# GuanRunwei/ASY-VRNet

Hardware: AMD Instinct MI355X
Metric: images/sec fwd+bwd, 512x512 img+4ch radar, bs=8/GPU (higher is better)
Workload: dtype f32; 1 GPU; EfficientVRNet(phi=l) forward+backward, 512x512 image + 4x512x512 radar, bs=8/GPU, fp32, det+seg heads (BASELINE.json configs[1]); random weights; global_batch=8, image_size=512, parallelism=dp1, launch=hipgraph

## Files before the change

asy-vrnet_amd/csrc/spatial.hip:

```cpp
#include "common.h"

#include <cstdlib>

namespace {

__global__ __launch_bounds__(256) void dwconv3x3_kernel(const float* x, long ldx, const float* w, float* y, long ldy,
                                                        int B, int H, int W, int C, int flip, int accumulate) {
  const int total = B * H * W * C;
  for (int e = blockIdx.x * 256 + threadIdx.x; e < total; e += gridDim.x * 256) {
    const int c = e % C;
    const int pix = e / C;
    const int xx = pix % W;
    const int q = pix / W;
    const int yy = q % H;
    const int b = q / H;
    float s = 0.f;
#pragma unroll
    for (int ky = 0; ky < 3; ++ky) {
      const int sy = yy + ky - 1;
      if (sy < 0 || sy >= H) continue;
      const float* row = x + ((long)(b * H + sy) * W) * ldx + c;
#pragma unroll
      for (int kx = 0; kx < 3; ++kx) {
        const int sx = xx + kx - 1;
// ... 223 lines not shown
    for (int j = 0; j < 4; ++j)
#pragma unroll
      for (int t = 0; t < 9; ++t) d[j * 9 + t] = acc[t][j];
  }
}
__global__ __launch_bounds__(256) void dwconv3x3_wgrad_reduce_kernel(const float* partial, int nchunks, int C, float* dw,
                                                                     int accumulate) {
  __shared__ double red[16][16];
  const int o = threadIdx.x & 15, sl = threadIdx.x >> 4;
  const int e = blockIdx.x * 16 + o;
  const bool live = e < C * 9;
  double s = 0;
  if (live)
    for (int k = sl; k < nchunks; k += 16) s += partial[(long)k * C * 9 + e];
  red[sl][o] = s;
  __syncthreads();
  if (sl == 0 && live) {
#pragma unroll
    for (int k = 1; k < 16; ++k) s += red[k][o];
    dw[e] = (accumulate ? dw[e] : 0.f) + (float)s;
  }
}

__global__ __launch_bounds__(256) void patch_gather_kernel(const float* x, long ldx, const float* pos, float* out, int B,
                                                           int H, int W, int C, int CP, int k) {
  const int CT = C + CP, KT = k * k * CT, OH = H / k, OW = W / k;
  const long total = (long)B * OH * OW * KT;
  for (long e = (long)blockIdx.x * 256 + threadIdx.x; e < total; e += (long)gridDim.x * 256) {
    const int ch = e % KT;
    const long op = e / KT;
    const int t = ch / CT, c = ch - t * CT;
    const int ky = t / k, kx = t - ky * k;
    const int ox = op % OW;
    const long q = op / OW;
    const int oy = q % OH;
    const long b = q / OH;
    const int yy = oy * k + ky, xx = ox * k + kx;
    out[e] = c < C ? x[((b * H + yy) * W + xx) * ldx + c] : pos[((long)yy * W + xx) * CP + (c - C)];
  }
}
__global__ __launch_bounds__(256) void patch_scatter_kernel(const float* dp, float* dx, long lddx, int B, int H, int W, int C,
                                                            int CP, int k, int accumulate) {
  const int CT = C + CP, KT = k * k * CT, OH = H / k, OW = W / k;
  const long total = (long)B * H * W * C;
  for (long e = (long)blockIdx.x * 256 + threadIdx.x; e < total; e += (long)gridDim.x * 256) {
    const int c = e % C;
    const long pix = e / C;
    const int xx = pix % W;
    const long q = pix / W;
    const int yy = q % H;
    const long b = q / H;
    const int t = (yy % k) * k + (xx % k);
    const float v = dp[((b * OH + yy / k) * OW + xx / k) * KT + t * CT + c];
    float* d = dx + pix * lddx + c;
    *d = accumulate ? *d + v : v;
  }
}
__global__ void ohwi_kernel(const float* src, float* dst, int Cout, int Cin, int T, int dir, int accumulate) {
  const long total = (long)Cout * Cin * T;
  const long e = (long)blockIdx.x * blockDim.x + threadIdx.x;
  if (e >= total) return;
  const int t = e % T;
  const long q = e / T;
  const int c = q % Cin;
  const long n = q / Cin;
  const long oihw = e, ohwi = (n * T + t) * Cin + c;
  if (dir == 0) dst[ohwi] = src[oihw];
  else dst[oihw] = (accumulate ? dst[oihw] : 0.f) + src[ohwi];
}

__device__ __forceinline__ void src_index(float scale, int o, int in_size, int* i0, int* i1, float* l1) {
  const float r = scale * (float)o;
  int a = (int)r;
  if (a > in_size - 1) a = in_size - 1;
  *i0 = a;
  *i1 = a + ((a < in_size - 1) ? 1 : 0);
  *l1 = r - (float)a;
}

__device__ __forceinline__ float up_tap(float v, const float* bnA, const float* bnD, const float* bnS, int c) {
  return bnA ? fmaxf(__builtin_fmaf(bnA[c], v - bnS[c], bnD[c]), 0.f) : v;
}

__global__ __launch_bounds__(256) void upsample_kernel(const float* x, long ldx, float* y, long ldy, int B, int H,
                                                       int W, int C, int OH, int OW, int out_nchw, const float* bnA,
                                                       const float* bnD, const float* bnS) {
  const float ry = OH > 1 ? (float)(H - 1) / (float)(OH - 1) : 0.f;
  const float rx = OW > 1 ? (float)(W - 1) / (float)(OW - 1) : 0.f;
  const long total = (long)B * OH * OW * C;
  for (long e = (long)blockIdx.x * 256 + threadIdx.x; e < total; e += (long)gridDim.x * 256) {
    int c, ox, oy;
    long b;
    if (out_nchw) {
      ox = e % OW; long q = e / OW; oy = q % OH; q /= OH; c = q % C; b = q / C;
    } else {
      c = e % C; long q = e / C; ox = q % OW; q /= OW; oy = q % OH; b = q / OH;
    }
    int y0, y1, x0, x1;
    float ly, lx;
    src_index(ry, oy, H, &y0, &y1, &ly);
    src_index(rx, ox, W, &x0, &x1, &lx);
    const float* base = x + (b * H * W) * ldx + c;
    const float v00 = up_tap(base[((long)y0 * W + x0) * ldx], bnA, bnD, bnS, c), v01 = up_tap(base[((long)y0 * W + x1) * ldx], bnA, bnD, bnS, c);
    const float v10 = up_tap(base[((long)y1 * W + x0) * ldx], bnA, bnD, bnS, c), v11 = up_tap(base[((long)y1 * W + x1) * ldx], bnA, bnD, bnS, c);
    const float v = (1.f - ly) * ((1.f - lx) * v00 + lx * v01) + ly * ((1.f - lx) * v10 + lx * v11);
    if (out_nchw) y[e] = v;
    else y[((b * OH + oy) * OW + ox) * ldy + c] = v;
  }
}

__global__ __launch_bounds__(256) void upsample_vec_kernel(const float* x, long ldx, float* y, long ldy, int B, int H, int W,
                                                           int C, int OH, int OW, const float* bnA, const float* bnD,
                                                           const float* bnS) {
  const float ry = OH > 1 ? (float)(H - 1) / (float)(OH - 1) : 0.f;
  const float rx = OW > 1 ? (float)(W - 1) / (float)(OW - 1) : 0.f;
  const int CQ = C >> 2;
  const long total = (long)B * OH * OW * CQ;
  for (long e = (long)blockIdx.x * 256 + threadIdx.x; e < total; e += (long)gridDim.x * 256) {
    const int cq = e % CQ;
    long q = e / CQ;
    const int ox = q % OW; q /= OW;
    const int oy = q % OH;
    const long b = q / OH;
    int y0, y1, x0, x1;
    float ly, lx;
    src_index(ry, oy, H, &y0, &y1, &ly);
    src_index(rx, ox, W, &x0, &x1, &lx);
    const float* base = x + (b * H * W) * ldx + 4 * cq;
    f32x4 v00 = *reinterpret_cast<const f32x4*>(base + ((long)y0 * W + x0) * ldx);
    f32x4 v01 = *reinterpret_cast<const f32x4*>(base + ((long)y0 * W + x1) * ldx);
    f32x4 v10 = *reinterpret_cast<const f32x4*>(base + ((long)y1 * W + x0) * ldx);
    f32x4 v11 = *reinterpret_cast<const f32x4*>(base + ((long)y1 * W + x1) * ldx);
    if (bnA) {
#pragma unroll
      for (int j = 0; j < 4; ++j) {
        const int c = 4 * cq + j;
        v00[j] = up_tap(v00[j], bnA, bnD, bnS, c);
        v01[j] = up_tap(v01[j], bnA, bnD, bnS, c);
        v10[j] = up_tap(v10[j], bnA, bnD, bnS, c);
        v11[j] = up_tap(v11[j], bnA, bnD, bnS, c);
      }
    }
    f32x4 v;
#pragma unroll
    for (int j = 0; j < 4; ++j) v[j] = (1.f - ly) * ((1.f - lx) * v00[j] + lx * v01[j]) + ly * ((1.f - lx) * v10[j] + lx * v11[j]);
    *reinterpret_cast<f32x4*>(y + ((b * OH + oy) * OW + ox) * ldy + 4 * cq) = v;
  }
}

__global__ __launch_bounds__(256) void upsample_bwd_vec_kernel(const float* dy, long lddy, float* dx, long lddx, int B, int H,
                                                               int W, int C, int OH, int OW, int accumulate) {
  const float ry = OH > 1 ? (float)(H - 1) / (float)(OH - 1) : 0.f;
  const float rx = OW > 1 ? (float)(W - 1) / (float)(OW - 1) : 0.f;
  const int CQ = C >> 2;
  const long total = (long)B * H * W * CQ;
  for (long e = (long)blockIdx.x * 256 + threadIdx.x; e < total; e += (long)gridDim.x * 256) {
    const int cq = e % CQ;
    long q = e / CQ;
    const int ix = q % W; q /= W;
    const int iy = q % H;
    const long b = q / H;
    int oy_lo = 0, oy_hi = OH - 1, ox_lo = 0, ox_hi = OW - 1;
    if (ry > 0.f) {
      oy_lo = max(0, (int)floorf((float)(iy - 1) / ry) - 1);
      oy_hi = min(OH - 1, (int)ceilf((float)(iy + 1) / ry) + 1);
    }
    if (rx > 0.f) {
      ox_lo = max(0, (int)floorf((float)(ix - 1) / rx) - 1);
      ox_hi = min(OW - 1, (int)ceilf((float)(ix + 1) / rx) + 1);
    }
    f32x4 s = {0.f, 0.f, 0.f, 0.f};
    for (int oy = oy_lo; oy <= oy_hi; ++oy) {
      int y0, y1;
      float ly;
      src_index(ry, oy, H, &y0, &y1, &ly);
      const float wy = (y0 == iy ? 1.f - ly : 0.f) + (y1 == iy ? ly : 0.f);
      if (wy == 0.f) continue;
      for (int ox = ox_lo; ox <= ox_hi; ++ox) {
        int x0, x1;
        float lx;
        src_index(rx, ox, W, &x0, &x1, &lx);
        const float wx = (x0 == ix ? 1.f - lx : 0.f) + (x1 == ix ? lx : 0.f);
        if (wx == 0.f) continue;
        const f32x4 g = *reinterpret_cast<const f32x4*>(dy + ((b * OH + oy) * (long)OW + ox) * lddy + 4 * cq);
        const float w = wy * wx;
#pragma unroll
        for (int j = 0; j < 4; ++j) s[j] += w * g[j];
      }
    }
    f32x4* d = reinterpret_cast<f32x4*>(dx + ((b * H + iy) * (long)W + ix) * lddx + 4 * cq);
    if (accumulate) s += *d;
    *d = s;
  }
}

__global__ __launch_bounds__(256) void upsample_nchw4_kernel(const float* x, long ldx, float* y, int B, int H, int W, int C,
                                                             int OH, int OW, const float* bnA, const float* bnD,
                                                             const float* bnS) {
  const float ry = OH > 1 ? (float)(H - 1) / (float)(OH - 1) : 0.f;
  const float rx = OW > 1 ? (float)(W - 1) / (float)(OW - 1) : 0.f;
  const int OQ = OW >> 2;
  const long total = (long)B * C * OH * OQ;
  for (long e = (long)blockIdx.x * 256 + threadIdx.x; e < total; e += (long)gridDim.x * 256) {
    const int oq = e % OQ;
    long q = e / OQ;
    const int oy = q % OH; q /= OH;
    const int c = q % C;
    const long b = q / C;
    int y0, y1;
    float ly;
    src_index(ry, oy, H, &y0, &y1, &ly);
    const float* r0 = x + ((b * H + y0) * (long)W) * ldx + c;
    const float* r1 = x + ((b * H + y1) * (long)W) * ldx + c;
    f32x4 v;
#pragma unroll
    for (int j = 0; j < 4; ++j) {
      int x0, x1;
      float lx;
      src_index(rx, 4 * oq + j, W, &x0, &x1, &lx);
      const float v00 = up_tap(r0[(long)x0 * ldx], bnA, bnD, bnS, c), v01 = up_tap(r0[(long)x1 * ldx], bnA, bnD, bnS, c);
      const float v10 = up_tap(r1[(long)x0 * ldx], bnA, bnD, bnS, c), v11 = up_tap(r1[(long)x1 * ldx], bnA, bnD, bnS, c);
      v[j] = (1.f - ly) * ((1.f - lx) * v00 + lx * v01) + ly * ((1.f - lx) * v10 + lx * v11);
    }
    *reinterpret_cast<f32x4*>(y + ((b * C + c) * OH + oy) * (long)OW + 4 * oq) = v;
  }
}

__global__ __launch_bounds__(256) void upsample_bwd_kernel(const float* dy, long lddy, int dy_nchw, float* dx, long lddx,
                                                           int B, int H, int W, int C, int OH, int OW, int accumulate) {
  const float ry = OH > 1 ? (float)(H - 1) / (float)(OH - 1) : 0.f;
  const float rx = OW > 1 ? (float)(W - 1) / (float)(OW - 1) : 0.f;
  const long total = (long)B * H * W * C;
  for (long e = (long)blockIdx.x * 256 + threadIdx.x; e < total; e += (long)gridDim.x * 256) {
    int c, ix, iy;
    long b;
    if (dy_nchw) {
      ix = e % W;
      long q = e / W;
      iy = q % H; q /= H;
      c = q % C;
      b = q / C;
    } else {
      c = e % C;
      long q = e / C;
      ix = q % W; q /= W;
      iy = q % H;
      b = q / H;
    }
    int oy_lo = 0, oy_hi = OH - 1, ox_lo = 0, ox_hi = OW - 1;
    if (ry > 0.f) {
      oy_lo = max(0, (int)floorf((float)(iy - 1) / ry) - 1);
      oy_hi = min(OH - 1, (int)ceilf((float)(iy + 1) / ry) + 1);
    }
    if (rx > 0.f) {
      ox_lo = max(0, (int)floorf((float)(ix - 1) / rx) - 1);
      ox_hi = min(OW - 1, (int)ceilf((float)(ix + 1) / rx) + 1);
    }
    float s = 0.f;
    constexpr int MAXR = 16;
    const int nx = ox_hi - ox_lo + 1;
    float wxs[MAXR];
    if (nx <= MAXR) {
#pragma unroll
      for (int t = 0; t < MAXR; ++t) {
        int x0, x1;
        float lx;
        src_index(rx, min(ox_lo + t, OW - 1), W, &x0, &x1, &lx);
        wxs[t] = t < nx ? (x0 == ix ? 1.f - lx : 0.f) + (x1 == ix ? lx : 0.f) : 0.f;
      }
    }
    for (int oy = oy_lo; oy <= oy_hi; ++oy) {
      int y0, y1;
      float ly;
      src_index(ry, oy, H, &y0, &y1, &ly);
      const float wy = (y0 == iy ? 1.f - ly : 0.f) + (y1 == iy ? ly : 0.f);
      if (wy == 0.f) continue;
      if (nx <= MAXR) {
        const float* grow = dy_nchw ? dy + ((b * C + c) * OH + oy) * (long)OW + ox_lo : dy + ((b * OH + oy) * (long)OW + ox_lo) * lddy + c;
        const long gstep = dy_nchw ? 1 : lddy;
#pragma unroll
        for (int t = 0; t < MAXR; ++t) {
          const float wx = wxs[t];
          if (wx == 0.f) continue;
          s += wy * wx * grow[t * gstep];
        }
        continue;
      }
      for (int ox = ox_lo; ox <= ox_hi; ++ox) {
        int x0, x1;
        float lx;
        src_index(rx, ox, W, &x0, &x1, &lx);
        const float wx = (x0 == ix ? 1.f - lx : 0.f) + (x1 == ix ? lx : 0.f);
        if (wx == 0.f) continue;
        const float g = dy_nchw ? dy[((b * C + c) * OH + oy) * (long)OW + ox]
                                : dy[((b * OH + oy) * (long)OW + ox) * lddy + c];
        s += wy * wx * g;
      }
    }
    float* d = dx + ((b * H + iy) * (long)W + ix) * lddx + c;
    *d = accumulate ? *d + s : s;
  }
}

__global__ __launch_bounds__(256) void minmax_partial_kernel(const float* p, long n, float* partial) {
  __shared__ float smn[4], smx[4];
  float mn = INFINITY, mx = -INFINITY;
  for (long e = (long)blockIdx.x * 256 + threadIdx.x; e < n; e += (long)gridDim.x * 256) {
    const float v = p[e];
    mn = fminf(mn, v);
    mx = fmaxf(mx, v);
  }
#pragma unroll
  for (int o = 32; o > 0; o >>= 1) {
    mn = fminf(mn, __shfl_xor(mn, o, 64));
    mx = fmaxf(mx, __shfl_xor(mx, o, 64));
  }
  if ((threadIdx.x & 63) == 0) {
    smn[threadIdx.x >> 6] = mn;
    smx[threadIdx.x >> 6] = mx;
  }
  __syncthreads();
  if (threadIdx.x == 0) {
    partial[2 * blockIdx.x] = fminf(fminf(smn[0], smn[1]), fminf(smn[2], smn[3]));
    partial[2 * blockIdx.x + 1] = fmaxf(fmaxf(smx[0], smx[1]), fmaxf(smx[2], smx[3]));
// ... 286 lines not shown
                                                           const float* P, const float* Q, const float* Mn, const float* E,
                                                           const float* F, float* dx, long lddx, long HW, int C,
                                                           int accumulate) {
  const long b = blockIdx.y;
  const long total = HW * C;
  for (long e = (long)blockIdx.x * 256 + threadIdx.x; e < total; e += (long)gridDim.x * 256) {
    const long r = e / C;
    const int q = e - r * C;
    const float xv = x[(b * HW + r) * ldx + q];
    const float pq = P[b * C + q], mq = Mn[b * C + q];
    const float sg = vr_sigmoid(pq * (xv - mq) + Q[b * C + q]);
    const float g = dy[(b * HW + r) * lddy + sa_dst(q, C)];
    const float v = g * (sg + xv * sg * (1.f - sg) * pq) + E[b * C + q] * (xv - mq) + F[b * C + q];
    float* d = dx + (b * HW + r) * lddx + q;
    *d = accumulate ? *d + v : v;
  }
}

inline long grid_for(long n, long per_block = 1024, long cap = 8192) {
  long g = vr_cdiv(n, per_block);
  return g < 1 ? 1 : (g > cap ? cap : g);
}

void sa_plan(long HW, int C, int* TPR, int* ncb, int* nchunks, long* rows) {
  int t = 1;
  while (t < C && t < 256) t <<= 1;
  *TPR = t;
  *ncb = (int)vr_cdiv(C, t);
  long nc = vr_cdiv(HW * C, 8192);
  if (nc < 1) nc = 1;
  if (nc > 1024) nc = 1024;
  if (nc > HW) nc = HW;
  *rows = vr_cdiv(HW, nc);
  *nchunks = (int)vr_cdiv(HW, *rows);
}

}

extern "C" int vrnet_dwconv3x3_f32(const float* x, long ldx, const float* w, float* y, long ldy, int B, int H, int W,
                                   int C, int flip, int accumulate, void* stream) {
  if (vr_ablated("dwconv")) return VR_OK;
  VR_CHECK_ARG(x && w && y && B > 0 && H > 0 && W > 0 && C > 0, "dwconv3x3: bad arguments");
  VR_CHECK_ARG((long)B * H * W * C < (1L << 31), "dwconv3x3: tensor too large");
  const bool vec = C % 4 == 0 && C <= 1024 && 256 % (C / 4) == 0 && ldx % 4 == 0 && ldy % 4 == 0 && vr_aligned16(x) &&
                   vr_aligned16(y) && vr_aligned16(w);
  static const int slide = vr_tune("VRNET_DW_SLIDE", 1);
// ... 49 lines not shown
    vr_set_error("dwconv3x3_wgrad: workspace too small");
    return VR_ERR_WORKSPACE;
  }
  const int TPR = C <= 32 ? 32 : 64;
  float* partial = reinterpret_cast<float*>(workspace);
  hipStream_t st = vr_stream(stream);
  if (dw_wgrad_slide_ok(W, C, ldx, lddy, x, dy) && vr_tune("VRNET_DW_WGRAD_SLIDE", 1)) {
    const int quads = C / 4 < 64 ? C / 4 : 64, groups = 256 / quads;
    hipLaunchKernelGGL(dwconv3x3_wgrad_slide_kernel, dim3(nchunks, (C / 4) / quads), dim3(256), (size_t)(groups - 1) * quads * 9 * 16, st,
                       x, ldx, dy, lddy, B, H, W, C, (int)ppc, partial);
  } else {
    hipLaunchKernelGGL(dwconv3x3_wgrad_kernel, dim3(nchunks, vr_cdiv(C, TPR)), dim3(256), 0, st, x, ldx, dy, lddy, B, H, W,
                       C, ppc, partial);
  }
  VR_LAUNCH_CHECK("dwconv3x3_wgrad");
  hipLaunchKernelGGL(dwconv3x3_wgrad_reduce_kernel, dim3(vr_cdiv(C * 9, 16)), dim3(256), 0, st, partial, nchunks, C, dw,
                     accumulate);
  VR_LAUNCH_CHECK("dwconv3x3_wgrad_reduce");
  return VR_OK;
}

static int upsample_launch(const float* x, long ldx, float* y, long ldy, int B, int H, int W, int C, int scale, int out_nchw,
                           const float* bnA, const float* bnD, const float* bnS, void* stream) {
  if (!out_nchw && C % 4 == 0 && ldx % 4 == 0 && ldy % 4 == 0 && vr_aligned16(x) && vr_aligned16(y))
    hipLaunchKernelGGL(upsample_vec_kernel, dim3(grid_for((long)B * H * W * scale * scale * (C / 4))), dim3(256), 0,
                       vr_stream(stream), x, ldx, y, ldy, B, H, W, C, H * scale, W * scale, bnA, bnD, bnS);
  else if (out_nchw && (W * scale) % 4 == 0 && vr_aligned16(y))
    hipLaunchKernelGGL(upsample_nchw4_kernel, dim3(grid_for((long)B * H * W * scale * scale * C / 4)), dim3(256), 0,
                       vr_stream(stream), x, ldx, y, B, H, W, C, H * scale, W * scale, bnA, bnD, bnS);
  else
    hipLaunchKernelGGL(upsample_kernel, dim3(grid_for((long)B * H * W * scale * scale * C)), dim3(256), 0,
                       vr_stream(stream), x, ldx, y, ldy, B, H, W, C, H * scale, W * scale, out_nchw, bnA, bnD, bnS);
  VR_LAUNCH_CHECK("upsample");
  return VR_OK;
}

extern "C" int vrnet_upsample_bilinear_f32(const float* x, long ldx, float* y, long ldy, int B, int H, int W, int C,
                                           int scale, int out_nchw, void* stream) {
  if (vr_ablated("misc")) return VR_OK;
  VR_CHECK_ARG(x && y && scale >= 1 && B > 0 && H > 0 && W > 0 && C > 0, "upsample: bad arguments");
  return upsample_launch(x, ldx, y, ldy, B, H, W, C, scale, out_nchw, nullptr, nullptr, nullptr, stream);
}

extern "C" int vrnet_bn_relu_upsample_bilinear_f32(const float* z, long ldz, const float* A, const float* D, const float* S,
                                                   float* y, long ldy, int B, int H, int W, int C, int scale, int out_nchw,
                                                   void* stream) {
  if (vr_ablated("misc")) return VR_OK;
  VR_CHECK_ARG(z && A && D && S && y && scale >= 1 && B > 0 && H > 0 && W > 0 && C > 0, "bn_relu_upsample: bad arguments");
  return upsample_launch(z, ldz, y, ldy, B, H, W, C, scale, out_nchw, A, D, S, stream);
}

extern "C" int vrnet_upsample_bilinear_bwd_f32(const float* dy, long lddy, int dy_nchw, float* dx, long lddx, int B,
                                               int H, int W, int C, int scale, int accumulate, void* stream) {
  if (vr_ablated("misc")) return VR_OK;
  VR_CHECK_ARG(dy && dx && scale >= 1, "upsample_bwd: bad arguments");
  if (!dy_nchw && C % 4 == 0 && lddy % 4 == 0 && lddx % 4 == 0 && vr_aligned16(dy) && vr_aligned16(dx))
    hipLaunchKernelGGL(upsample_bwd_vec_kernel, dim3(grid_for((long)B * H * W * (C / 4), 256)), dim3(256), 0, vr_stream(stream),
                       dy, lddy, dx, lddx, B, H, W, C, H * scale, W * scale, accumulate);
  else
    hipLaunchKernelGGL(upsample_bwd_kernel, dim3(grid_for((long)B * H * W * C, 256)), dim3(256), 0, vr_stream(stream), dy,
                       lddy, dy_nchw, dx, lddx, B, H, W, C, H * scale, W * scale, accumulate);
  VR_LAUNCH_CHECK("upsample_bwd");
  return VR_OK;
}

extern "C" long vrnet_reduce_workspace(void) { return 8192L * 4 * 8 + 256; }

extern "C" int vrnet_minmax_f32(const float* p, long n, float* mm, void* workspace, long workspace_bytes, void* stream) {
  VR_CHECK_ARG(p && mm && workspace && n > 0, "minmax: bad arguments");
  VR_CHECK_ARG(workspace_bytes >= vrnet_reduce_workspace(), "minmax: workspace too small");
  const int nb = (int)grid_for(n, 2048, 2048);
  float* partial = reinterpret_cast<float*>(workspace);
  hipLaunchKernelGGL(minmax_partial_kernel, dim3(nb), dim3(256), 0, vr_stream(stream), p, n, partial);
  VR_LAUNCH_CHECK("minmax_partial");
  hipLaunchKernelGGL(minmax_final_kernel, dim3(1), dim3(256), 0, vr_stream(stream), partial, nb, mm);
  VR_LAUNCH_CHECK("minmax_final");
  return VR_OK;
}

extern "C" int vrnet_enhance_mul_f32(const float* p, const float* x, const float* mm, float* out, long n, void* stream) {
  VR_CHECK_ARG(p && x && mm && out && n > 0, "enhance_mul: bad arguments");
  hipLaunchKernelGGL(enhance_mul_kernel, dim3(grid_for(n)), dim3(256), 0, vr_stream(stream), p, x, mm, out, n);
  VR_LAUNCH_CHECK("enhance_mul");
  return VR_OK;
// ... 77 lines not shown
  hipLaunchKernelGGL(sa_bwd_reduce_kernel, dim3(nchunks, B, ncb), dim3(256), 256 * 2 * sizeof(double), st, dy, lddy, x,
                     ldx, P, Q, Mn, HW, C, TPR, rows, nchunks, partial);
  VR_LAUNCH_CHECK("sa_bwd_reduce");
  hipLaunchKernelGGL(sa_reduce_chunks_kernel, dim3(vr_cdiv((long)B * C * 2, 16)), dim3(256), 0, st, partial, T, B,
                     nchunks, C);
  VR_LAUNCH_CHECK("sa_reduce_chunks");
  SaParams sp{cw, cb, sw, sb, gnw, gnb};
  const int nb1 = (int)vr_cdiv((long)B * C, 256);
  float* E = EF;
  float* F = EF + (long)B * C;
  hipLaunchKernelGGL(sa_coef_bwd_kernel, dim3(nb1 + C / (2 * G)), dim3(256), 0, st, T, mom, sp, B, HW, C, G, nb1, E, F, dcw, dcb,
                     dsw, dsb, dgnw, dgnb, accumulate_params);
  VR_LAUNCH_CHECK("sa_coef_bwd");
  hipLaunchKernelGGL(sa_bwd_apply_kernel, dim3(grid_for(HW * C), B), dim3(256), 0, st, dy, lddy, x, ldx, P, Q, Mn, E, F, dx,
                     lddx, HW, C, accumulate_dx);
  VR_LAUNCH_CHECK("sa_bwd_apply");
  return VR_OK;
}

extern "C" int vrnet_patch_gather_f32(const float* x, long ldx, const float* pos, float* out, int B, int H, int W, int C,
                                      int CP, int k, void* stream) {
  VR_CHECK_ARG(x && out && (CP == 0 || pos) && B > 0 && C > 0 && CP >= 0 && k > 0 && H % k == 0 && W % k == 0 && ldx >= C,
               "patch_gather: bad arguments");
  hipLaunchKernelGGL(patch_gather_kernel, dim3(grid_for((long)B * H * W * (C + CP))), dim3(256), 0, vr_stream(stream), x,
                     ldx, pos, out, B, H, W, C, CP, k);
  VR_LAUNCH_CHECK("patch_gather");
  return VR_OK;
}

extern "C" int vrnet_patch_scatter_f32(const float* dp, float* dx, long lddx, int B, int H, int W, int C, int CP, int k,
                                       int accumulate, void* stream) {
  VR_CHECK_ARG(dp && dx && B > 0 && C > 0 && CP >= 0 && k > 0 && H % k == 0 && W % k == 0 && lddx >= C,
               "patch_scatter: bad arguments");
  hipLaunchKernelGGL(patch_scatter_kernel, dim3(grid_for((long)B * H * W * C)), dim3(256), 0, vr_stream(stream), dp, dx,
                     lddx, B, H, W, C, CP, k, accumulate);
  VR_LAUNCH_CHECK("patch_scatter");
  return VR_OK;
}

extern "C" int vrnet_weight_ohwi_f32(const float* src, float* dst, int Cout, int Cin, int kh, int kw, int dir,
                                     int accumulate, void* stream) {
  VR_CHECK_ARG(src && dst && Cout > 0 && Cin > 0 && kh > 0 && kw > 0 && (dir == 0 || dir == 1), "weight_ohwi: bad arguments");
  const long total = (long)Cout * Cin * kh * kw;
  hipLaunchKernelGGL(ohwi_kernel, dim3(vr_cdiv(total, 256)), dim3(256), 0, vr_stream(stream), src, dst, Cout, Cin, kh * kw,
                     dir, accumulate);
  VR_LAUNCH_CHECK("weight_ohwi");
  return VR_OK;
}
```

asy-vrnet_amd/csrc/tinyconv.hip:

```cpp
#include "common.h"

namespace tiny {

constexpr int CMAX = 8;

struct Args {
  const float* a; long lda; const float* w; const float* bias; float* y; long ldy;
  int B, H, W, Cin, Cout, k, pad, dil, accumulate;
};

template <int MODE>
__global__ __launch_bounds__(256) void conv_kernel(const Args p) {
  __shared__ float ws[9 * CMAX * CMAX];
  const int T = p.k * p.k;
  for (int i = threadIdx.x; i < T * p.Cout * p.Cin; i += 256) ws[i] = p.w[i];
  __syncthreads();
  const int CK = MODE == 0 ? p.Cin : p.Cout, CN = MODE == 0 ? p.Cout : p.Cin;
  const long total = (long)p.B * p.H * p.W;
  for (long pix = (long)blockIdx.x * 256 + threadIdx.x; pix < total; pix += (long)gridDim.x * 256) {
    const int x = pix % p.W;
    const long q = pix / p.W;
    const int y = q % p.H;
    const long b = q / p.H;
    float acc[CMAX];
// ... 224 lines not shown
  for (int n = 0; n < NO; ++n) {
#pragma unroll
    for (int c = 0; c < CP; ++c)
#pragma unroll
      for (int t = 0; t < T; ++t) {
        const float sum = row16(acc[n][c][t]);
        if (lead) red[rowid][n * NA + c * T + t] = sum;
      }
    const float b = row16(bs[n]);
    if (lead) red[rowid][n * NA + CP * T] = b;
  }
  __syncthreads();
  const int per = Cin * T + 1;
  for (int i = threadIdx.x; i < NO * per; i += 256) {
    const int n = i / per, j = i - n * per;
    const int src = n * NA + (j == Cin * T ? CP * T : j);
    float sum = 0.f;
#pragma unroll
    for (int r = 0; r < 16; ++r) sum += red[r][src];
    partial[((long)blockIdx.x * NO + n) * per + j] = sum;
  }
}

__global__ __launch_bounds__(256) void wgrad_reduce_kernel(const float* partial, int nblk, int Cin, int Cout, int T,
                                                           const float* row_scale, float* dw, float* db, int accumulate) {
  __shared__ double red[16][16];
  const int per = Cin * T + 1;
  const int o = threadIdx.x & 15, sl = threadIdx.x >> 4;
  const int e = blockIdx.x * 16 + o;
  const bool live = e < Cout * per;
  const int n = live ? e / per : 0, i = e - n * per;
  double s = 0;
  if (live)
    for (int b = sl; b < nblk; b += 16) s += partial[((long)b * Cout + n) * per + i];
  red[sl][o] = s;
  __syncthreads();
  if (sl != 0 || !live) return;
#pragma unroll
  for (int k = 1; k < 16; ++k) s += red[k][o];
  float v = (float)s;
  if (row_scale) v *= row_scale[n];
  if (i == Cin * T) {
    if (db) db[n] = accumulate ? db[n] + v : v;
  } else {
    float* d = dw + (long)n * Cin * T + i;
    *d = accumulate ? *d + v : v;
  }
}

__global__ __launch_bounds__(256) void patch_dgrad_kernel(const float* dy, long lddy, const float* w, float* dx, long lddx,
                                                          int B, int H, int W, int Cin, int Cout, int k, int accumulate) {
  extern __shared__ float wsm[];
  const int T = k * k;
  for (int i = threadIdx.x; i < T * Cout * Cin; i += 256) wsm[i] = w[i];
  __syncthreads();
  const int OW = W / k, OH = H / k;
  const long total = (long)B * H * W;
  for (long pix = (long)blockIdx.x * 256 + threadIdx.x; pix < total; pix += (long)gridDim.x * 256) {
    const int x = pix % W;
    const long q = pix / W;
    const int y = q % H;
    const long b = q / H;
    const int t = (y % k) * k + (x % k);
// ... 29 lines not shown
    VR_LAUNCH_CHECK("tiny_conv");                                                                                  \
    return VR_OK;                                                                                                  \
  } while (0)
  if (al && mode == 0) {
    if (Cin == 3 && Cout == 3 && k == 1) VR_TINY_FIXED(0, 3, 3, 1);
    if (Cin == 4 && Cout == 4 && k == 1) VR_TINY_FIXED(0, 4, 4, 1);
    if (Cin == 7 && Cout == 4 && k == 1) VR_TINY_FIXED(0, 7, 4, 1);
    if (Cin == 4 && Cout == 3 && k == 3) VR_TINY_FIXED(0, 4, 3, 3);
  } else if (al) {
    if (Cin == 7 && Cout == 4 && k == 1) VR_TINY_FIXED(1, 4, 7, 1);
    if (Cin == 4 && Cout == 3 && k == 3) VR_TINY_FIXED(1, 3, 4, 3);
    if (Cin == 4 && Cout == 4 && k == 1) VR_TINY_FIXED(1, 4, 4, 1);
    if (Cin == 3 && Cout == 3 && k == 1) VR_TINY_FIXED(1, 3, 3, 1);
  }
#undef VR_TINY_FIXED
  if (mode == 0) hipLaunchKernelGGL((tiny::conv_kernel<0>), dim3(blocks), dim3(256), 0, st, p);
  else hipLaunchKernelGGL((tiny::conv_kernel<1>), dim3(blocks), dim3(256), 0, st, p);
  VR_LAUNCH_CHECK("tiny_conv");
  return VR_OK;
}

static void tiny_wgrad_plan(long npix, int* nblk, long* ppb) {
  long nb = vr_cdiv(npix, 1024);
  if (nb > 2048) nb = 2048;
  if (nb < 1) nb = 1;
  *ppb = vr_cdiv(npix, nb);
  *nblk = (int)vr_cdiv(npix, *ppb);
}

long vr_tiny_wgrad_workspace(long npix, int Cin, int Cout, int T) {
  int nblk;
  long ppb;
  tiny_wgrad_plan(npix, &nblk, &ppb);
  return (long)nblk * Cout * (Cin * T + 1) * 4 + 256;
}

int vr_tiny_wgrad(const float* x, long ldx, const float* dy, long lddy, float* dw, float* db, const float* row_scale,
                  int B, int H, int W, int Cin, int Cout, int k, int pad, int dil, int accumulate, void* workspace,
                  hipStream_t st) {
  int nblk;
  long ppb;
  tiny_wgrad_plan((long)B * H * W, &nblk, &ppb);
  float* partial = reinterpret_cast<float*>(workspace);
  const int vec4 = Cin == 4 && ldx % 4 == 0 && vr_aligned16(x);
  dim3 grid(nblk, Cout), block(256);
#define VR_TINY_WGRAD_ALL(CP_, KS_, NO_)                                                                                 \
  do {                                                                                                                   \
    hipLaunchKernelGGL((tiny::wgrad_all_kernel<CP_, KS_, NO_>), dim3(nblk), block, 0, st, x, ldx, dy, lddy, B, H, W, Cin, pad, \
                       dil, vec4, ppb, partial);                                                                         \
    goto reduce;                                                                                                         \
  } while (0)
  if (k == 3 && Cin == 4 && Cout == 3) VR_TINY_WGRAD_ALL(4, 3, 3);
  if (k == 1 && Cin == 7 && Cout == 4) VR_TINY_WGRAD_ALL(8, 1, 4);
  if (k == 1 && Cin == 4 && Cout == 4) VR_TINY_WGRAD_ALL(4, 1, 4);
  if (k == 1 && Cin == 3 && Cout == 3) VR_TINY_WGRAD_ALL(4, 1, 3);
#undef VR_TINY_WGRAD_ALL
#define VR_TINY_WGRAD(CP_, KS_)                                                                                          \
  hipLaunchKernelGGL((tiny::wgrad_kernel<CP_, KS_>), grid, block, 0, st, x, ldx, dy, lddy, B, H, W, Cin, Cout, pad, dil, vec4, \
                     ppb, partial)
  if (k == 1) {
    if (Cin <= 4) VR_TINY_WGRAD(4, 1);
    else VR_TINY_WGRAD(8, 1);
  } else {
    if (Cin <= 4) VR_TINY_WGRAD(4, 3);
    else VR_TINY_WGRAD(8, 3);
  }
#undef VR_TINY_WGRAD
reduce:
  VR_LAUNCH_CHECK("tiny_wgrad");
  const int per = Cin * k * k + 1;
  hipLaunchKernelGGL(tiny::wgrad_reduce_kernel, dim3(vr_cdiv(Cout * per, 16)), dim3(256), 0, st, partial, nblk, Cin, Cout,
                     k * k, row_scale, dw, db, accumulate);
  VR_LAUNCH_CHECK("tiny_wgrad_reduce");
  return VR_OK;
}

int vr_patch_dgrad(const float* dy, long lddy, const float* w, float* dx, long lddx, int B, int H, int W, int Cin,
                   int Cout, int k, int accumulate, hipStream_t st) {
  long blocks = vr_cdiv((long)B * H * W, 256);
  if (blocks > 16384) blocks = 16384;
  const size_t lds = (size_t)k * k * Cout * Cin * sizeof(float);
  hipLaunchKernelGGL(tiny::patch_dgrad_kernel, dim3(blocks), dim3(256), lds, st, dy, lddy, w, dx, lddx, B, H, W, Cin, Cout,
                     k, accumulate);
  VR_LAUNCH_CHECK("patch_dgrad");
  return VR_OK;
}
```

Baseline: 326.3 images/sec.

## Row-structured indexing for upsample/patch kernels and block-per-output wgrad reduce

Replaces flat grid-stride loops with 64-bit div/mod decomposition in the patch gather/scatter and bilinear upsample forward/backward kernels by a row/item iteration helper that uses 32-bit unsigned index math and fewer divisions. The upsample backward kernels also tighten the contributing output range by trimming zero-weight taps, cache horizontal weights in a smaller fixed array, and use FMA. The tiny-conv weight-gradient reduce now assigns one block per output element, with a wave-level sum instead of a 16x16 shared-memory layout. The point is to cut integer-division overhead and improve coalescing. In exchange it adds argument checks limiting sizes to 2^31 elements and changes floating-point rounding through the explicit FMA usage.

```diff
diff --git a/asy-vrnet_amd/csrc/spatial.hip b/asy-vrnet_amd/csrc/spatial.hip
--- a/asy-vrnet_amd/csrc/spatial.hip
+++ b/asy-vrnet_amd/csrc/spatial.hip
@@ -269,39 +269,47 @@
   }
 }
 
+template <int IPT = 4, class F>
+__device__ __forceinline__ void for_row_items(unsigned rows, unsigned n, F f) {
+  constexpr unsigned CH = 256 * IPT;
+  const unsigned rp = n >= 256 ? 1 : 256 / n;
+  const unsigned nc = (n + CH - 1) / CH;
+  const unsigned sub = threadIdx.x / n, i0 = threadIdx.x - sub * n;
+  if (sub >= rp) return;
+  const unsigned nblk = ((rows + rp - 1) / rp) * nc;
+  for (unsigned blk = blockIdx.x; blk < nblk; blk += gridDim.x) {
+    const unsigned rg = blk / nc, chunk = blk - rg * nc;
+    const unsigned row = rg * rp + sub;
+    if (row >= rows) continue;
+    const unsigned i1 = min(n, (chunk + 1) * CH);
+    for (unsigned i = chunk * CH + i0; i < i1; i += 256) f(row, i);
+  }
+}
+
 __global__ __launch_bounds__(256) void patch_gather_kernel(const float* x, long ldx, const float* pos, float* out, int B,
                                                            int H, int W, int C, int CP, int k) {
-  const int CT = C + CP, KT = k * k * CT, OH = H / k, OW = W / k;
-  const long total = (long)B * OH * OW * KT;
-  for (long e = (long)blockIdx.x * 256 + threadIdx.x; e < total; e += (long)gridDim.x * 256) {
-    const int ch = e % KT;
-    const long op = e / KT;
-    const int t = ch / CT, c = ch - t * CT;
-    const int ky = t / k, kx = t - ky * k;
-    const int ox = op % OW;
-    const long q = op / OW;
-    const int oy = q % OH;
-    const long b = q / OH;
-    const int yy = oy * k + ky, xx = ox * k + kx;
-    out[e] = c < C ? x[((b * H + yy) * W + xx) * ldx + c] : pos[((long)yy * W + xx) * CP + (c - C)];
-  }
+  const unsigned CT = C + CP, KT = k * k * CT, OH = H / k, OW = W / k;
+  for_row_items(B * OH, OW * KT, [&](unsigned row, unsigned i) {
+    const unsigned b = row / OH, oy = row - b * OH;
+    const unsigned ox = i / KT, ch = i - ox * KT;
+    const unsigned t = ch / CT, c = ch - t * CT;
+    const unsigned ky = t / k, kx = t - ky * k;
+    const unsigned yy = oy * k + ky, xx = ox * k + kx;
+    out[(long)row * (OW * KT) + i] = c < (unsigned)C ? x[(((long)b * H + yy) * W + xx) * ldx + c] : pos[((long)yy * W + xx) * CP + (c - C)];
+  });
 }
 __global__ __launch_bounds__(256) void patch_scatter_kernel(const float* dp, float* dx, long lddx, int B, int H, int W, int C,
                                                             int CP, int k, int accumulate) {
-  const int CT = C + CP, KT = k * k * CT, OH = H / k, OW = W / k;
-  const long total = (long)B * H * W * C;
-  for (long e = (long)blockIdx.x * 256 + threadIdx.x; e < total; e += (long)gridDim.x * 256) {
-    const int c = e % C;
-    const long pix = e / C;
-    const int xx = pix % W;
-    const long q = pix / W;
-    const int yy = q % H;
-    const long b = q / H;
-    const int t = (yy % k) * k + (xx % k);
-    const float v = dp[((b * OH + yy / k) * OW + xx / k) * KT + t * CT + c];
-    float* d = dx + pix * lddx + c;
+  const unsigned CT = C + CP, KT = k * k * CT, OH = H / k, OW = W / k;
+  for_row_items(B * H, W * C, [&](unsigned row, unsigned i) {
+    const unsigned b = row / H, yy = row - b * H;
+    const unsigned xx = i / C, c = i - xx * C;
+    const unsigned oy = yy / k, ox = xx / k;
+    const unsigned t = (yy - oy * k) * k + (xx - ox * k);
+    const float v = dp[(((long)b * OH + oy) * OW + ox) * KT + t * CT + c];
+    float* d = dx + ((long)row * W + xx) * lddx + c;
     *d = accumulate ? *d + v : v;
-  }
+  });
 }
 __global__ void ohwi_kernel(const float* src, float* dst, int Cout, int Cin, int T, int dir, int accumulate) {
   const long total = (long)Cout * Cin * T;
@@ -316,13 +324,21 @@
   else dst[oihw] = (accumulate ? dst[oihw] : 0.f) + src[ohwi];
 }
 
+template <bool FUSED>
 __device__ __forceinline__ void src_index(float scale, int o, int in_size, int* i0, int* i1, float* l1) {
+#pragma clang fp contract(off)
   const float r = scale * (float)o;
   int a = (int)r;
   if (a > in_size - 1) a = in_size - 1;
   *i0 = a;
   *i1 = a + ((a < in_size - 1) ? 1 : 0);
-  *l1 = r - (float)a;
+  *l1 = FUSED ? __builtin_fmaf(scale, (float)o, -(float)a) : r - (float)a;
+}
+__device__ __forceinline__ float up_blend(float ly, float lx, float v00, float v01, float v10, float v11) {
+#pragma clang fp contract(off)
+  const float top = __builtin_fmaf(1.f - lx, v00, lx * v01);
+  const float bot = __builtin_fmaf(1.f - lx, v10, lx * v11);
+  return __builtin_fmaf(1.f - ly, top, ly * bot);
 }
 
 __device__ __forceinline__ float up_tap(float v, const float* bnA, const float* bnD, const float* bnS, int c) {
@@ -334,26 +350,25 @@
                                                        const float* bnD, const float* bnS) {
   const float ry = OH > 1 ? (float)(H - 1) / (float)(OH - 1) : 0.f;
   const float rx = OW > 1 ? (float)(W - 1) / (float)(OW - 1) : 0.f;
-  const long total = (long)B * OH * OW * C;
-  for (long e = (long)blockIdx.x * 256 + threadIdx.x; e < total; e += (long)gridDim.x * 256) {
-    int c, ox, oy;
-    long b;
+  for_row_items(out_nchw ? B * C * OH : B * OH, out_nchw ? OW : OW * C, [&](unsigned row, unsigned i) {
+    unsigned c, ox, oy, b;
     if (out_nchw) {
-      ox = e % OW; long q = e / OW; oy = q % OH; q /= OH; c = q % C; b = q / C;
+      const unsigned q = row / OH;
+      oy = row - q * OH; b = q / C; c = q - b * C; ox = i;
     } else {
-      c = e % C; long q = e / C; ox = q % OW; q /= OW; oy = q % OH; b = q / OH;
+      b = row / OH; oy = row - b * OH; ox = i / C; c = i - ox * C;
     }
     int y0, y1, x0, x1;
     float ly, lx;
-    src_index(ry, oy, H, &y0, &y1, &ly);
-    src_index(rx, ox, W, &x0, &x1, &lx);
-    const float* base = x + (b * H * W) * ldx + c;
+    src_index<false>(ry, oy, H, &y0, &y1, &ly);
+    src_index<false>(rx, ox, W, &x0, &x1, &lx);
+    const float* base = x + ((long)b * H * W) * ldx + c;
     const float v00 = up_tap(base[((long)y0 * W + x0) * ldx], bnA, bnD, bnS, c), v01 = up_tap(base[((long)y0 * W + x1) * ldx], bnA, bnD, bnS, c);
     const float v10 = up_tap(base[((long)y1 * W + x0) * ldx], bnA, bnD, bnS, c), v11 = up_tap(base[((long)y1 * W + x1) * ldx], bnA, bnD, bnS, c);
-    const float v = (1.f - ly) * ((1.f - lx) * v00 + lx * v01) + ly * ((1.f - lx) * v10 + lx * v11);
-    if (out_nchw) y[e] = v;
-    else y[((b * OH + oy) * OW + ox) * ldy + c] = v;
-  }
+    const float v = up_blend(ly, lx, v00, v01, v10, v11);
+    if (out_nchw) y[(long)row * OW + ox] = v;
+    else y[((long)row * OW + ox) * ldy + c] = v;
+  });
 }
 
 __global__ __launch_bounds__(256) void upsample_vec_kernel(const float* x, long ldx, float* y, long ldy, int B, int H, int W,
@@ -361,19 +376,15 @@
                                                            const float* bnS) {
   const float ry = OH > 1 ? (float)(H - 1) / (float)(OH - 1) : 0.f;
   const float rx = OW > 1 ? (float)(W - 1) / (float)(OW - 1) : 0.f;
-  const int CQ = C >> 2;
-  const long total = (long)B * OH * OW * CQ;
-  for (long e = (long)blockIdx.x * 256 + threadIdx.x; e < total; e += (long)gridDim.x * 256) {
-    const int cq = e % CQ;
-    long q = e / CQ;
-    const int ox = q % OW; q /= OW;
-    const int oy = q % OH;
-    const long b = q / OH;
+  const unsigned CQ = C >> 2;
+  for_row_items(B * OH, OW * CQ, [&](unsigned row, unsigned i) {
+    const unsigned b = row / OH, oy = row - b * OH;
+    const unsigned ox = i / CQ, cq = i - ox * CQ;
     int y0, y1, x0, x1;
     float ly, lx;
-    src_index(ry, oy, H, &y0, &y1, &ly);
-    src_index(rx, ox, W, &x0, &x1, &lx);
-    const float* base = x + (b * H * W) * ldx + 4 * cq;
+    src_index<false>(ry, oy, H, &y0, &y1, &ly);
+    src_index<false>(rx, ox, W, &x0, &x1, &lx);
+    const float* base = x + ((long)b * H * W) * ldx + 4 * cq;
     f32x4 v00 = *reinterpret_cast<const f32x4*>(base + ((long)y0 * W + x0) * ldx);
     f32x4 v01 = *reinterpret_cast<const f32x4*>(base + ((long)y0 * W + x1) * ldx);
     f32x4 v10 = *reinterpret_cast<const f32x4*>(base + ((long)y1 * W + x0) * ldx);
@@ -390,55 +401,79 @@
     }
     f32x4 v;
 #pragma unroll
-    for (int j = 0; j < 4; ++j) v[j] = (1.f - ly) * ((1.f - lx) * v00[j] + lx * v01[j]) + ly * ((1.f - lx) * v10[j] + lx * v11[j]);
-    *reinterpret_cast<f32x4*>(y + ((b * OH + oy) * OW + ox) * ldy + 4 * cq) = v;
-  }
-}
+    for (int j = 0; j < 4; ++j) v[j] = up_blend(ly, lx, v00[j], v01[j], v10[j], v11[j]);
+    *reinterpret_cast<f32x4*>(y + ((long)row * OW + ox) * ldy + 4 * cq) = v;
+  });
+}
+
+__device__ __forceinline__ float up_weight(float scale, int o, int in_size, int in) {
+  int i0, i1;
+  float l;
+  src_index<true>(scale, o, in_size, &i0, &i1, &l);
+  return (i0 == in ? 1.f - l : 0.f) + (i1 == in ? l : 0.f);
+}
+__device__ __forceinline__ void up_range(float scale, int in, int in_size, int out_size, int* lo, int* hi) {
+  int a = 0, b = out_size - 1;
+  if (scale > 0.f) {
+    a = max(0, (int)floorf((float)(in - 1) / scale) - 1);
+    b = min(out_size - 1, (int)ceilf((float)(in + 1) / scale) + 1);
+  }
+  while (a < b && up_weight(scale, a, in_size, in) == 0.f) ++a;
+  while (b > a && up_weight(scale, b, in_size, in) == 0.f) --b;
+  *lo = a;
+  *hi = b;
+}
+constexpr int UP_MAXR = 12;
 
 __global__ __launch_bounds__(256) void upsample_bwd_vec_kernel(const float* dy, long lddy, float* dx, long lddx, int B, int H,
                                                                int W, int C, int OH, int OW, int accumulate) {
   const float ry = OH > 1 ? (float)(H - 1) / (float)(OH - 1) : 0.f;
   const float rx = OW > 1 ? (float)(W - 1) / (float)(OW - 1) : 0.f;
-  const int CQ = C >> 2;
-  const long total = (long)B * H * W * CQ;
-  for (long e = (long)blockIdx.x * 256 + threadIdx.x; e < total; e += (long)gridDim.x * 256) {
-    const int cq = e % CQ;
-    long q = e / CQ;
-    const int ix = q % W; q /= W;
-    const int iy = q % H;
-    const long b = q / H;
-    int oy_lo = 0, oy_hi = OH - 1, ox_lo = 0, ox_hi = OW - 1;
-    if (ry > 0.f) {
-      oy_lo = max(0, (int)floorf((float)(iy - 1) / ry) - 1);
-      oy_hi = min(OH - 1, (int)ceilf((float)(iy + 1) / ry) + 1);
-    }
-    if (rx > 0.f) {
-      ox_lo = max(0, (int)floorf((float)(ix - 1) / rx) - 1);
-      ox_hi = min(OW - 1, (int)ceilf((float)(ix + 1) / rx) + 1);
+  const unsigned CQ = C >> 2;
+  for_row_items<1>(B * H, W * CQ, [&](unsigned row, unsigned i) {
+    const unsigned b = row / H;
+    const int iy = row - b * H;
+    const unsigned uix = i / CQ, cq = i - uix * CQ;
+    const int ix = uix;
+    int oy_lo, oy_hi, ox_lo, ox_hi;
+    up_range(ry, iy, H, OH, &oy_lo, &oy_hi);
+    up_range(rx, ix, W, OW, &ox_lo, &ox_hi);
+    const int nx = ox_hi - ox_lo + 1;
+    float wxs[UP_MAXR];
+    if (nx <= UP_MAXR) {
+#pragma unroll
+      for (int t = 0; t < UP_MAXR; ++t) wxs[t] = t < nx ? up_weight(rx, min(ox_lo + t, OW - 1), W, ix) : 0.f;
     }
     f32x4 s = {0.f, 0.f, 0.f, 0.f};
     for (int oy = oy_lo; oy <= oy_hi; ++oy) {
-      int y0, y1;
-      float ly;
-      src_index(ry, oy, H, &y0, &y1, &ly);
-      const float wy = (y0 == iy ? 1.f - ly : 0.f) + (y1 == iy ? ly : 0.f);
+      const float wy = up_weight(ry, oy, H, iy);
       if (wy == 0.f) continue;
+      const float* grow = dy + (((long)b * OH + oy) * (long)OW + ox_lo) * lddy + 4 * cq;
+      if (nx <= UP_MAXR) {
+#pragma unroll
+        for (int t = 0; t < UP_MAXR; ++t) {
+          const float wx = wxs[t];
+          if (wx == 0.f) continue;
+          const f32x4 g = *reinterpret_cast<const f32x4*>(grow + t * lddy);
+          const float w = wy * wx;
+#pragma unroll
+          for (int j = 0; j < 4; ++j) s[j] = __builtin_fmaf(w, g[j], s[j]);
+        }
+        continue;
+      }
       for (int ox = ox_lo; ox <= ox_hi; ++ox) {
-        int x0, x1;
-        float lx;
-        src_index(rx, ox, W, &x0, &x1, &lx);
-        const float wx = (x0 == ix ? 1.f - lx : 0.f) + (x1 == ix ? lx : 0.f);
+        const float wx = up_weight(rx, ox, W, ix);
         if (wx == 0.f) continue;
-        const f32x4 g = *reinterpret_cast<const f32x4*>(dy + ((b * OH + oy) * (long)OW + ox) * lddy + 4 * cq);
+        const f32x4 g = *reinterpret_cast<const f32x4*>(grow + (long)(ox - ox_lo) * lddy);
         const float w = wy * wx;
 #pragma unroll
-        for (int j = 0; j < 4; ++j) s[j] += w * g[j];
-      }
-    }
-    f32x4* d = reinterpret_cast<f32x4*>(dx + ((b * H + iy) * (long)W + ix) * lddx + 4 * cq);
+        for (int j = 0; j < 4; ++j) s[j] = __builtin_fmaf(w, g[j], s[j]);
+      }
+    }
+    f32x4* d = reinterpret_cast<f32x4*>(dx + ((long)row * W + ix) * lddx + 4 * cq);
     if (accumulate) s += *d;
     *d = s;
-  }
+  });
 }
 
 __global__ __launch_bounds__(256) void upsample_nchw4_kernel(const float* x, long ldx, float* y, int B, int H, int W, int C,
@@ -446,107 +481,76 @@
                                                              const float* bnS) {
   const float ry = OH > 1 ? (float)(H - 1) / (float)(OH - 1) : 0.f;
   const float rx = OW > 1 ? (float)(W - 1) / (float)(OW - 1) : 0.f;
-  const int OQ = OW >> 2;
-  const long total = (long)B * C * OH * OQ;
-  for (long e = (long)blockIdx.x * 256 + threadIdx.x; e < total; e += (long)gridDim.x * 256) {
-    const int oq = e % OQ;
-    long q = e / OQ;
-    const int oy = q % OH; q /= OH;
-    const int c = q % C;
-    const long b = q / C;
+  for_row_items(B * C * OH, OW >> 2, [&](unsigned row, unsigned oq) {
+    const unsigned q = row / OH, oy = row - q * OH;
+    const unsigned b = q / C, c = q - b * C;
     int y0, y1;
     float ly;
-    src_index(ry, oy, H, &y0, &y1, &ly);
-    const float* r0 = x + ((b * H + y0) * (long)W) * ldx + c;
-    const float* r1 = x + ((b * H + y1) * (long)W) * ldx + c;
+    src_index<false>(ry, oy, H, &y0, &y1, &ly);
+    const float* r0 = x + (((long)b * H + y0) * (long)W) * ldx + c;
+    const float* r1 = x + (((long)b * H + y1) * (long)W) * ldx + c;
     f32x4 v;
 #pragma unroll
     for (int j = 0; j < 4; ++j) {
       int x0, x1;
       float lx;
-      src_index(rx, 4 * oq + j, W, &x0, &x1, &lx);
+      src_index<false>(rx, 4 * oq + j, W, &x0, &x1, &lx);
       const float v00 = up_tap(r0[(long)x0 * ldx], bnA, bnD, bnS, c), v01 = up_tap(r0[(long)x1 * ldx], bnA, bnD, bnS, c);
       const float v10 = up_tap(r1[(long)x0 * ldx], bnA, bnD, bnS, c), v11 = up_tap(r1[(long)x1 * ldx], bnA, bnD, bnS, c);
-      v[j] = (1.f - ly) * ((1.f - lx) * v00 + lx * v01) + ly * ((1.f - lx) * v10 + lx * v11);
-    }
-    *reinterpret_cast<f32x4*>(y + ((b * C + c) * OH + oy) * (long)OW + 4 * oq) = v;
-  }
+      v[j] = up_blend(ly, lx, v00, v01, v10, v11);
+    }
+    *reinterpret_cast<f32x4*>(y + (long)row * OW + 4 * oq) = v;
+  });
 }
 
 __global__ __launch_bounds__(256) void upsample_bwd_kernel(const float* dy, long lddy, int dy_nchw, float* dx, long lddx,
                                                            int B, int H, int W, int C, int OH, int OW, int accumulate) {
   const float ry = OH > 1 ? (float)(H - 1) / (float)(OH - 1) : 0.f;
   const float rx = OW > 1 ? (float)(W - 1) / (float)(OW - 1) : 0.f;
-  const long total = (long)B * H * W * C;
-  for (long e = (long)blockIdx.x * 256 + threadIdx.x; e < total; e += (long)gridDim.x * 256) {
-    int c, ix, iy;
-    long b;
+  for_row_items<1>(dy_nchw ? B * C * H : B * H, dy_nchw ? W : W * C, [&](unsigned row, unsigned i) {
+    unsigned c, b;
+    int ix, iy;
     if (dy_nchw) {
-      ix = e % W;
-      long q = e / W;
-      iy = q % H; q /= H;
-      c = q % C;
-      b = q / C;
+      const unsigned q = row / H;
+      iy = row - q * H; b = q / C; c = q - b * C; ix = i;
     } else {
-      c = e % C;
-      long q = e / C;
-      ix = q % W; q /= W;
-      iy = q % H;
-      b = q / H;
-    }
-    int oy_lo = 0, oy_hi = OH - 1, ox_lo = 0, ox_hi = OW - 1;
-    if (ry > 0.f) {
-      oy_lo = max(0, (int)floorf((float)(iy - 1) / ry) - 1);
-      oy_hi = min(OH - 1, (int)ceilf((float)(iy + 1) / ry) + 1);
-    }
-    if (rx > 0.f) {
-      ox_lo = max(0, (int)floorf((float)(ix - 1) / rx) - 1);
-      ox_hi = min(OW - 1, (int)ceilf((float)(ix + 1) / rx) + 1);
-    }
+      b = row / H; iy = row - b * H;
+      const unsigned uix = i / C;
+      ix = uix; c = i - uix * C;
+    }
+    int oy_lo, oy_hi, ox_lo, ox_hi;
+    up_range(ry, iy, H, OH, &oy_lo, &oy_hi);
+    up_range(rx, ix, W, OW, &ox_lo, &ox_hi);
     float s = 0.f;
-    constexpr int MAXR = 16;
     const int nx = ox_hi - ox_lo + 1;
-    float wxs[MAXR];
-    if (nx <= MAXR) {
-#pragma unroll
-      for (int t = 0; t < MAXR; ++t) {
-        int x0, x1;
-        float lx;
-        src_index(rx, min(ox_lo + t, OW - 1), W, &x0, &x1, &lx);
-        wxs[t] = t < nx ? (x0 == ix ? 1.f - lx : 0.f) + (x1 == ix ? lx : 0.f) : 0.f;
-      }
+    float wxs[UP_MAXR];
+    if (nx <= UP_MAXR) {
+#pragma unroll
+      for (int t = 0; t < UP_MAXR; ++t) wxs[t] = t < nx ? up_weight(rx, min(ox_lo + t, OW - 1), W, ix) : 0.f;
     }
     for (int oy = oy_lo; oy <= oy_hi; ++oy) {
-      int y0, y1;
-      float ly;
-      src_index(ry, oy, H, &y0, &y1, &ly);
-      const float wy = (y0 == iy ? 1.f - ly : 0.f) + (y1 == iy ? ly : 0.f);
+      const float wy = up_weight(ry, oy, H, iy);
       if (wy == 0.f) continue;
-      if (nx <= MAXR) {
-        const float* grow = dy_nchw ? dy + ((b * C + c) * OH + oy) * (long)OW + ox_lo : dy + ((b * OH + oy) * (long)OW + ox_lo) * lddy + c;
-        const long gstep = dy_nchw ? 1 : lddy;
-#pragma unroll
-        for (int t = 0; t < MAXR; ++t) {
+      const float* grow = dy_nchw ? dy + (((long)b * C + c) * OH + oy) * (long)OW + ox_lo : dy + (((long)b * OH + oy) * (long)OW + ox_lo) * lddy + c;
+      const long gstep = dy_nchw ? 1 : lddy;
+      if (nx <= UP_MAXR) {
+#pragma unroll
+        for (int t = 0; t < UP_MAXR; ++t) {
           const float wx = wxs[t];
           if (wx == 0.f) continue;
-          s += wy * wx * grow[t * gstep];
+          s = __builtin_fmaf(wy * wx, grow[t * gstep], s);
         }
         continue;
       }
       for (int ox = ox_lo; ox <= ox_hi; ++ox) {
-        int x0, x1;
-        float lx;
-        src_index(rx, ox, W, &x0, &x1, &lx);
-        const float wx = (x0 == ix ? 1.f - lx : 0.f) + (x1 == ix ? lx : 0.f);
+        const float wx = up_weight(rx, ox, W, ix);
         if (wx == 0.f) continue;
-        const float g = dy_nchw ? dy[((b * C + c) * OH + oy) * (long)OW + ox]
-                                : dy[((b * OH + oy) * (long)OW + ox) * lddy + c];
-        s += wy * wx * g;
-      }
-    }
-    float* d = dx + ((b * H + iy) * (long)W + ix) * lddx + c;
+        s = __builtin_fmaf(wy * wx, grow[(ox - ox_lo) * gstep], s);
+      }
+    }
+    float* d = dx + (dy_nchw ? (((long)b * H + iy) * (long)W + ix) : ((long)row * W + ix)) * lddx + c;
     *d = accumulate ? *d + s : s;
-  }
+  });
 }
 
 __global__ __launch_bounds__(256) void minmax_partial_kernel(const float* p, long n, float* partial) {
@@ -879,6 +883,13 @@
   return g < 1 ? 1 : (g > cap ? cap : g);
 }
 
+inline bool row_items_ok(long rows, long n) { return rows > 0 && n > 0 && rows * n < (1L << 31); }
+inline long row_items_grid(long rows, long n, int ipt = 4, long cap = 65536) {
+  const long rp = n >= 256 ? 1 : 256 / n, nc = vr_cdiv(n, 256L * ipt);
+  const long g = vr_cdiv(rows, rp) * nc;
+  return g > cap ? cap : g;
+}
+
 void sa_plan(long HW, int C, int* TPR, int* ncb, int* nchunks, long* rows) {
   int t = 1;
   while (t < C && t < 256) t <<= 1;
@@ -974,15 +985,17 @@
 
 static int upsample_launch(const float* x, long ldx, float* y, long ldy, int B, int H, int W, int C, int scale, int out_nchw,
                            const float* bnA, const float* bnD, const float* bnS, void* stream) {
+  const long OH = (long)H * scale, OW = (long)W * scale;
+  VR_CHECK_ARG(row_items_ok((long)B * OH, OW * C), "upsample: more than 2^31 output elements");
   if (!out_nchw && C % 4 == 0 && ldx % 4 == 0 && ldy % 4 == 0 && vr_aligned16(x) && vr_aligned16(y))
-    hipLaunchKernelGGL(upsample_vec_kernel, dim3(grid_for((long)B * H * W * scale * scale * (C / 4))), dim3(256), 0,
-                       vr_stream(stream), x, ldx, y, ldy, B, H, W, C, H * scale, W * scale, bnA, bnD, bnS);
-  else if (out_nchw && (W * scale) % 4 == 0 && vr_aligned16(y))
-    hipLaunchKernelGGL(upsample_nchw4_kernel, dim3(grid_for((long)B * H * W * scale * scale * C / 4)), dim3(256), 0,
-                       vr_stream(stream), x, ldx, y, B, H, W, C, H * scale, W * scale, bnA, bnD, bnS);
+    hipLaunchKernelGGL(upsample_vec_kernel, dim3(row_items_grid(B * OH, OW * (C / 4))), dim3(256), 0,
+                       vr_stream(stream), x, ldx, y, ldy, B, H, W, C, (int)OH, (int)OW, bnA, bnD, bnS);
+  else if (out_nchw && OW % 4 == 0 && vr_aligned16(y))
+    hipLaunchKernelGGL(upsample_nchw4_kernel, dim3(row_items_grid(B * C * OH, OW / 4)), dim3(256), 0,
+                       vr_stream(stream), x, ldx, y, B, H, W, C, (int)OH, (int)OW, bnA, bnD, bnS);
   else
-    hipLaunchKernelGGL(upsample_kernel, dim3(grid_for((long)B * H * W * scale * scale * C)), dim3(256), 0,
-                       vr_stream(stream), x, ldx, y, ldy, B, H, W, C, H * scale, W * scale, out_nchw, bnA, bnD, bnS);
+    hipLaunchKernelGGL(upsample_kernel, dim3(out_nchw ? row_items_grid(B * C * OH, OW) : row_items_grid(B * OH, OW * C)), dim3(256), 0,
+                       vr_stream(stream), x, ldx, y, ldy, B, H, W, C, (int)OH, (int)OW, out_nchw, bnA, bnD, bnS);
   VR_LAUNCH_CHECK("upsample");
   return VR_OK;
 }
@@ -1005,13 +1018,14 @@
 extern "C" int vrnet_upsample_bilinear_bwd_f32(const float* dy, long lddy, int dy_nchw, float* dx, long lddx, int B,
                                                int H, int W, int C, int scale, int accumulate, void* stream) {
   if (vr_ablated("misc")) return VR_OK;
-  VR_CHECK_ARG(dy && dx && scale >= 1, "upsample_bwd: bad arguments");
+  VR_CHECK_ARG(dy && dx && scale >= 1 && B > 0 && H > 0 && W > 0 && C > 0, "upsample_bwd: bad arguments");
+  VR_CHECK_ARG(row_items_ok((long)B * H * scale, (long)W * scale * C), "upsample_bwd: more than 2^31 gradient elements");
   if (!dy_nchw && C % 4 == 0 && lddy % 4 == 0 && lddx % 4 == 0 && vr_aligned16(dy) && vr_aligned16(dx))
-    hipLaunchKernelGGL(upsample_bwd_vec_kernel, dim3(grid_for((long)B * H * W * (C / 4), 256)), dim3(256), 0, vr_stream(stream),
+    hipLaunchKernelGGL(upsample_bwd_vec_kernel, dim3(row_items_grid((long)B * H, (long)W * (C / 4), 1)), dim3(256), 0, vr_stream(stream),
                        dy, lddy, dx, lddx, B, H, W, C, H * scale, W * scale, accumulate);
   else
-    hipLaunchKernelGGL(upsample_bwd_kernel, dim3(grid_for((long)B * H * W * C, 256)), dim3(256), 0, vr_stream(stream), dy,
-                       lddy, dy_nchw, dx, lddx, B, H, W, C, H * scale, W * scale, accumulate);
+    hipLaunchKernelGGL(upsample_bwd_kernel, dim3(dy_nchw ? row_items_grid((long)B * C * H, W, 1) : row_items_grid((long)B * H, (long)W * C, 1)),
+                       dim3(256), 0, vr_stream(stream), dy, lddy, dy_nchw, dx, lddx, B, H, W, C, H * scale, W * scale, accumulate);
   VR_LAUNCH_CHECK("upsample_bwd");
   return VR_OK;
 }
@@ -1135,8 +1149,9 @@
                                       int CP, int k, void* stream) {
   VR_CHECK_ARG(x && out && (CP == 0 || pos) && B > 0 && C > 0 && CP >= 0 && k > 0 && H % k == 0 && W % k == 0 && ldx >= C,
                "patch_gather: bad arguments");
-  hipLaunchKernelGGL(patch_gather_kernel, dim3(grid_for((long)B * H * W * (C + CP))), dim3(256), 0, vr_stream(stream), x,
-                     ldx, pos, out, B, H, W, C, CP, k);
+  VR_CHECK_ARG(row_items_ok((long)B * H, (long)W * (C + CP)), "patch_gather: more than 2^31 elements");
+  hipLaunchKernelGGL(patch_gather_kernel, dim3(row_items_grid((long)B * (H / k), (long)(W / k) * k * k * (C + CP))), dim3(256), 0,
+                     vr_stream(stream), x, ldx, pos, out, B, H, W, C, CP, k);
   VR_LAUNCH_CHECK("patch_gather");
   return VR_OK;
 }
@@ -1145,7 +1160,8 @@
                                        int accumulate, void* stream) {
   VR_CHECK_ARG(dp && dx && B > 0 && C > 0 && CP >= 0 && k > 0 && H % k == 0 && W % k == 0 && lddx >= C,
                "patch_scatter: bad arguments");
-  hipLaunchKernelGGL(patch_scatter_kernel, dim3(grid_for((long)B * H * W * C)), dim3(256), 0, vr_stream(stream), dp, dx,
+  VR_CHECK_ARG(row_items_ok((long)B * H, (long)W * (C + CP)), "patch_scatter: more than 2^31 elements");
+  hipLaunchKernelGGL(patch_scatter_kernel, dim3(row_items_grid((long)B * H, (long)W * C)), dim3(256), 0, vr_stream(stream), dp, dx,
                      lddx, B, H, W, C, CP, k, accumulate);
   VR_LAUNCH_CHECK("patch_scatter");
   return VR_OK;
diff --git a/asy-vrnet_amd/csrc/tinyconv.hip b/asy-vrnet_amd/csrc/tinyconv.hip
--- a/asy-vrnet_amd/csrc/tinyconv.hip
+++ b/asy-vrnet_amd/csrc/tinyconv.hip
@@ -270,23 +270,28 @@
   }
 }
 
+constexpr int WGRAD_MAX_BLOCKS = 2048;
 __global__ __launch_bounds__(256) void wgrad_reduce_kernel(const float* partial, int nblk, int Cin, int Cout, int T,
                                                            const float* row_scale, float* dw, float* db, int accumulate) {
-  __shared__ double red[16][16];
+  __shared__ double red[4];
   const int per = Cin * T + 1;
-  const int o = threadIdx.x & 15, sl = threadIdx.x >> 4;
-  const int e = blockIdx.x * 16 + o;
-  const bool live = e < Cout * per;
-  const int n = live ? e / per : 0, i = e - n * per;
+  const int e = blockIdx.x;
+  const int n = e / per, i = e - n * per;
+  const long stride = (long)Cout * per;
+  float v8[WGRAD_MAX_BLOCKS / 256];
+#pragma unroll
+  for (int j = 0; j < WGRAD_MAX_BLOCKS / 256; ++j) {
+    const int b = threadIdx.x + 256 * j;
+    v8[j] = b < nblk ? partial[b * stride + e] : 0.f;
+  }
   double s = 0;
-  if (live)
-    for (int b = sl; b < nblk; b += 16) s += partial[((long)b * Cout + n) * per + i];
-  red[sl][o] = s;
-  __syncthreads();
-  if (sl != 0 || !live) return;
-#pragma unroll
-  for (int k = 1; k < 16; ++k) s += red[k][o];
-  float v = (float)s;
+#pragma unroll
+  for (int j = 0; j < WGRAD_MAX_BLOCKS / 256; ++j) s += (double)v8[j];
+  s = wave_sum(s);
+  if ((threadIdx.x & 63) == 0) red[threadIdx.x >> 6] = s;
+  __syncthreads();
+  if (threadIdx.x != 0) return;
+  float v = (float)(((red[0] + red[1]) + red[2]) + red[3]);
   if (row_scale) v *= row_scale[n];
   if (i == Cin * T) {
     if (db) db[n] = accumulate ? db[n] + v : v;
@@ -362,7 +367,7 @@
 
 static void tiny_wgrad_plan(long npix, int* nblk, long* ppb) {
   long nb = vr_cdiv(npix, 1024);
-  if (nb > 2048) nb = 2048;
+  if (nb > tiny::WGRAD_MAX_BLOCKS) nb = tiny::WGRAD_MAX_BLOCKS;
   if (nb < 1) nb = 1;
   *ppb = vr_cdiv(npix, nb);
   *nblk = (int)vr_cdiv(npix, *ppb);
@@ -409,7 +414,7 @@
 reduce:
   VR_LAUNCH_CHECK("tiny_wgrad");
   const int per = Cin * k * k + 1;
-  hipLaunchKernelGGL(tiny::wgrad_reduce_kernel, dim3(vr_cdiv(Cout * per, 16)), dim3(256), 0, st, partial, nblk, Cin, Cout,
+  hipLaunchKernelGGL(tiny::wgrad_reduce_kernel, dim3(Cout * per), dim3(256), 0, st, partial, nblk, Cin, Cout,
                      k * k, row_scale, dw, db, accumulate);
   VR_LAUNCH_CHECK("tiny_wgrad_reduce");
   return VR_OK;
```

Measured after the change: 328.3 images/sec, median of 6. No clear change (+0.6%).
